# nnanhuang/S3Gaussian

Measured on AMD Instinct MI355X. Metric: train_iters_per_sec, higher is better.
Workload: dtype f32

## Files before the change

include/s3g_loss.h:

```cpp
#ifndef S3G_LOSS_H
#define S3G_LOSS_H
#ifdef __cplusplus
extern "C" {
#endif

#ifndef S3G_SUM_SLOTS
#define S3G_SUM_SLOTS 64
#define S3G_SUM_STRIDE 16
#define S3G_SUM_DOUBLES (S3G_SUM_SLOTS * S3G_SUM_STRIDE)
#endif

int s3g_ssim_forward(int C, int H, int W, const float* img1, const float* img2, double* ssim_sum, float* dm_dmu1,
                     float* dm_dsigma1_sq, float* dm_dsigma12, void* stream);

int s3g_ssim_backward(int C, int H, int W, const float* img1, const float* img2, const float* dm_dmu1,
                      const float* dm_dsigma1_sq, const float* dm_dsigma12, const float* dL_dmean, float* dL_dimg1,
                      void* stream);

typedef struct s3g_plane_reg_desc {
  const float* plane;
  float* grad;
  int H, W;
  float w_smooth, w_l1;
} s3g_plane_reg_desc;

#define S3G_MAX_REG_PLANES 48
int s3g_plane_regulation(int nplanes, const s3g_plane_reg_desc* planes, double* value, void* stream);

int s3g_scale_unless_one(float* x, size_t n, const float* scale , void* stream);

int s3g_pixel_losses_forward(int H, int W, const float* image, const float* gt_image, const float* depth,
                             const float* gt_depth, const float* feat, const float* gt_feat, float max_depth,
                             double* sums, void* stream);

int s3g_pixel_losses_combine(int H, int W, const double* sums, double* totals, float w_l1, float w_depth, float w_ssim,
                             float w_feat, float* loss, void* stream);

int s3g_pixel_losses_backward(int H, int W, const float* image, const float* gt_image, const float* depth,
                              const float* gt_depth, const float* feat, const float* gt_feat, float max_depth,
                              const double* totals, const float* g, float w_l1, float w_depth, float w_feat,
                              float* g_image, int accumulate_image, float* g_depth, float* g_feat, void* stream);

#ifdef __cplusplus
}
#endif
#endif
```

s3gaussian_amd/_lib.py:

```python
from __future__ import annotations

import ctypes as C
import os
import subprocess

_HERE = os.path.dirname(os.path.abspath(__file__))
LIB_PATH = os.environ.get("S3G_LIB_PATH") or os.path.join(_HERE, "lib", "libs3g.so")
CSRC_DIR = os.path.join(_HERE, "csrc")

ABI_VERSION = 16

RESIZE_FN = C.CFUNCTYPE(C.c_void_p, C.c_void_p, C.c_size_t)


class RasterInputs(C.Structure):
    _fields_ = [
        ("P", C.c_int), ("D", C.c_int), ("M", C.c_int), ("width", C.c_int), ("height", C.c_int),
        ("background", C.c_void_p), ("means3D", C.c_void_p), ("shs", C.c_void_p), ("colors_precomp", C.c_void_p),
        ("opacities", C.c_void_p), ("scales", C.c_void_p), ("scale_modifier", C.c_float), ("rotations", C.c_void_p),
        ("cov3D_precomp", C.c_void_p), ("viewmatrix", C.c_void_p), ("projmatrix", C.c_void_p), ("cam_pos", C.c_void_p),
        ("tan_fovx", C.c_float), ("tan_fovy", C.c_float), ("prefiltered", C.c_int), ("debug", C.c_int),
    ]


# ... 89 lines not shown
    return _torch.cuda.current_stream().cuda_stream


class _NullContext:
    __slots__ = ()

    def __enter__(self):
        return None

    def __exit__(self, *exc):
        return False


_NULL = _NullContext()


def on_device(dev):
    global _torch, _raw_stream, _cur_device
    if _torch is None:
        _torch, _raw_stream, _cur_device = _bind_fast_paths()
    if _cur_device is not None and getattr(dev, "index", None) is not None and _cur_device() == dev.index:
        return _NULL
    return _torch.cuda.device(dev)


def check(code: int) -> None:
    if code != 0:
        msg = lib().s3g_last_error().decode("utf-8", "replace")
        if code == 1:
            raise Exception(msg)
        raise RuntimeError(f"libs3g error {code}: {msg}")


EXPORTED_SYMBOLS = ["s3g_raster_forward", "s3g_raster_forward_reuse", "s3g_raster_forward_decompose", "s3g_raster_forward2", "s3g_raster_forward_async", "s3g_raster_arena_bytes", "s3g_adam_step_guarded", "s3g_raster_backward", "s3g_raster_backward_workspace_bytes", "s3g_raster_backward2", "s3g_raster_backward2_workspace_bytes", "s3g_hexplane_forward_workspace_bytes", "s3g_knn_workspace_bytes", "s3g_knn_mean_dist2", "s3g_hexplane_forward", "s3g_hexplane_backward", "s3g_hexplane_backward_algo", "s3g_hexplane_backward_workspace_bytes", "s3g_hexplane_backward_scratch_rows", "s3g_hexplane_debug_walk_mask", "s3g_hexplane_set_deterministic", "s3g_hexplane_get_deterministic", "s3g_hexplane_sort_state_words", "s3g_profile_enable", "s3g_profile_read", "s3g_ssim_forward", "s3g_ssim_backward", "s3g_plane_regulation", "s3g_scale_unless_one", "s3g_pixel_losses_forward", "s3g_pixel_losses_combine", "s3g_pixel_losses_backward", "s3g_glue_forward", "s3g_glue_backward", "s3g_deform_mlp_forward", "s3g_deform_mlp_backward", "s3g_deform_mlp_backward_ordered", "s3g_deform_mlp_wgrad_partial_bytes", "s3g_deform_mlp_stash_bytes", "s3g_deform_mlp_pack_bytes", "s3g_deform_mlp_set_arithmetic", "s3g_deform_mlp_get_arithmetic", "s3g_deform_infer", "s3g_deform_infer_split", "s3g_deform_infer_workspace_bytes", "s3g_adam_step", "s3g_densify_stats", "s3g_densify_stats_guarded", "s3g_density_count_words", "s3g_density_classify_densify", "s3g_density_classify_prune", "s3g_density_scan", "s3g_density_apply", "s3g_density_reset_opacity", "s3g_image_metrics_workspace_bytes", "s3g_image_metrics", "s3g_scene_flow_workspace_bytes", "s3g_scene_flow_colors", "s3g_frame_workspace_bytes", "s3g_frame_tiles", "s3g_split_count_words", "s3g_split_workspace_bytes", "s3g_split_classify", "s3g_split_mask_offsets", "s3g_split_pack_rows", "s3g_raster_backward_accum", "s3g_raster_backward2_accum", "s3g_mark_visible", "s3g_raster_set_exact_cull", "s3g_raster_get_exact_cull", "s3g_raster_set_bin_band", "s3g_raster_set_backward_wave_bounds", "s3g_last_error", "s3g_abi_version"]
```

s3gaussian_amd/csrc/ssim.hip:

```cpp
#include "common.hpp"

#include "../../include/s3g_loss.h"

namespace s3g {

constexpr int SS_T = 16, SS_R = 5, SS_H = SS_T + 2 * SS_R;

struct SsimWindow {
  float g[11];
};
static SsimWindow make_window() {
  SsimWindow w;
  float s = 0.f;
  for (int x = 0; x < 11; x++) {
    w.g[x] = (float)exp(-(double)((x - 5) * (x - 5)) / (2.0 * 1.5 * 1.5));
    s += w.g[x];
  }
  for (int x = 0; x < 11; x++) w.g[x] /= s;
  return w;
}

__global__ void __launch_bounds__(256) ssim_forward_kernel(int C, int H, int W, const float* __restrict__ img1,
                                                           const float* __restrict__ img2, const SsimWindow win,
                                                           double* __restrict__ ssim_sum, float* __restrict__ m_mu1,
                                                           float* __restrict__ m_s11, float* __restrict__ m_s12) {
  __shared__ float t1[SS_H][SS_H + 1], t2[SS_H][SS_H + 1];
  __shared__ float hb[5][SS_H][SS_T + 1];
  __shared__ float red[4];
  const int c = blockIdx.z, x0 = blockIdx.x * SS_T, y0 = blockIdx.y * SS_T;
  const int tid = threadIdx.x, lx = tid & 15, ly = tid >> 4;
  const size_t plane = (size_t)c * H * W;
  for (int i = tid; i < SS_H * SS_H; i += 256) {
    const int r = i / SS_H, q = i - r * SS_H;
    const int gy = y0 + r - SS_R, gx = x0 + q - SS_R;
    const bool in = gy >= 0 && gy < H && gx >= 0 && gx < W;
    t1[r][q] = in ? img1[plane + (size_t)gy * W + gx] : 0.f;
    t2[r][q] = in ? img2[plane + (size_t)gy * W + gx] : 0.f;
  }
  __syncthreads();
  for (int i = tid; i < SS_H * SS_T; i += 256) {
    const int r = i / SS_T, q = i - r * SS_T;
    float a = 0.f, b = 0.f, aa = 0.f, bb = 0.f, ab = 0.f;
#pragma unroll
    for (int k = 0; k < 11; k++) {
      const float w = win.g[k], u = t1[r][q + k], v = t2[r][q + k];
      a += w * u; b += w * v; aa += w * (u * u); bb += w * (v * v); ab += w * (u * v);
    }
    hb[0][r][q] = a; hb[1][r][q] = b; hb[2][r][q] = aa; hb[3][r][q] = bb; hb[4][r][q] = ab;
  }
  __syncthreads();
  float mu1 = 0.f, mu2 = 0.f, e11 = 0.f, e22 = 0.f, e12 = 0.f;
#pragma unroll
  for (int k = 0; k < 11; k++) {
    const float w = win.g[k];
    mu1 += w * hb[0][ly + k][lx]; mu2 += w * hb[1][ly + k][lx]; e11 += w * hb[2][ly + k][lx];
    e22 += w * hb[3][ly + k][lx]; e12 += w * hb[4][ly + k][lx];
  }
  const int gx = x0 + lx, gy = y0 + ly;
  float val = 0.f;
  if (gx < W && gy < H) {
    const float C1 = 0.01f * 0.01f, C2 = 0.03f * 0.03f;
    const float mu1_sq = mu1 * mu1, mu2_sq = mu2 * mu2, mu12 = mu1 * mu2;
    const float s11 = e11 - mu1_sq, s22 = e22 - mu2_sq, s12 = e12 - mu12;
    const float a = 2.f * mu12 + C1, b = 2.f * s12 + C2, cc = mu1_sq + mu2_sq + C1, d = s11 + s22 + C2;
    const float inv = 1.f / (cc * d);
    val = (a * b) * inv;
    const float dm_ds11 = -val / d;
    const float dm_ds12 = 2.f * a * inv;
    const float dm_dmu1 = 2.f * mu2 * b * inv - 2.f * mu1 * val / cc + dm_ds11 * (-2.f * mu1) + dm_ds12 * (-mu2);
    const size_t o = plane + (size_t)gy * W + gx;
    m_mu1[o] = dm_dmu1; m_s11[o] = dm_ds11; m_s12[o] = dm_ds12;
  }
  for (int off = 32; off >= 1; off >>= 1) val += __shfl_xor(val, off);
  if ((tid & 63) == 0) red[tid >> 6] = val;
  __syncthreads();
  if (tid == 0) {
    const unsigned b = blockIdx.x + gridDim.x * (blockIdx.y + gridDim.y * blockIdx.z);
    atomicAdd(&ssim_sum[(b % S3G_SUM_SLOTS) * S3G_SUM_STRIDE], (double)(red[0] + red[1] + red[2] + red[3]));
  }
}

__global__ void __launch_bounds__(256) ssim_backward_kernel(int C, int H, int W, const float* __restrict__ img1,
                                                            const float* __restrict__ img2, const SsimWindow win,
                                                            const float* __restrict__ m_mu1, const float* __restrict__ m_s11,
                                                            const float* __restrict__ m_s12, const float* __restrict__ dL_dmean,
                                                            float* __restrict__ dL_dimg1) {
  __shared__ float t[3][SS_H][SS_H + 1];
  __shared__ float hb[3][SS_H][SS_T + 1];
  const int c = blockIdx.z, x0 = blockIdx.x * SS_T, y0 = blockIdx.y * SS_T;
  const int tid = threadIdx.x, lx = tid & 15, ly = tid >> 4;
  const size_t plane = (size_t)c * H * W;
  for (int i = tid; i < SS_H * SS_H; i += 256) {
    const int r = i / SS_H, q = i - r * SS_H;
    const int gy = y0 + r - SS_R, gx = x0 + q - SS_R;
    const bool in = gy >= 0 && gy < H && gx >= 0 && gx < W;
    const size_t o = plane + (size_t)gy * W + gx;
    t[0][r][q] = in ? m_mu1[o] : 0.f;
    t[1][r][q] = in ? m_s11[o] : 0.f;
    t[2][r][q] = in ? m_s12[o] : 0.f;
  }
  __syncthreads();
  for (int i = tid; i < SS_H * SS_T; i += 256) {
    const int r = i / SS_T, q = i - r * SS_T;
    float a = 0.f, b = 0.f, d = 0.f;
#pragma unroll
    for (int k = 0; k < 11; k++) {
      const float w = win.g[k];
      a += w * t[0][r][q + k]; b += w * t[1][r][q + k]; d += w * t[2][r][q + k];
    }
    hb[0][r][q] = a; hb[1][r][q] = b; hb[2][r][q] = d;
  }
  __syncthreads();
  float A = 0.f, B = 0.f, D = 0.f;
#pragma unroll
  for (int k = 0; k < 11; k++) {
    const float w = win.g[k];
    A += w * hb[0][ly + k][lx]; B += w * hb[1][ly + k][lx]; D += w * hb[2][ly + k][lx];
  }
  const int gx = x0 + lx, gy = y0 + ly;
  if (gx < W && gy < H) {
    const size_t o = plane + (size_t)gy * W + gx;
    const float scale = dL_dmean[0] / (float)((size_t)C * H * W);
    dL_dimg1[o] = scale * (A + 2.f * img1[o] * B + img2[o] * D);
  }
}

}

using namespace s3g;

extern "C" int s3g_ssim_forward(int C, int H, int W, const float* img1, const float* img2, double* ssim_sum, float* dm_dmu1,
                                float* dm_dsigma1_sq, float* dm_dsigma12, void* stream_) {
  if (C <= 0 || H <= 0 || W <= 0 || !img1 || !img2 || !ssim_sum || !dm_dmu1 || !dm_dsigma1_sq || !dm_dsigma12) {
    set_error("s3g_ssim_forward: bad argument");
    return S3G_ERR_INVALID_ARG;
  }
  static const SsimWindow win = make_window();
  dim3 grid((W + SS_T - 1) / SS_T, (H + SS_T - 1) / SS_T, C);
  hipLaunchKernelGGL(ssim_forward_kernel, grid, dim3(256), 0, (hipStream_t)stream_, C, H, W, img1, img2, win, ssim_sum,
                     dm_dmu1, dm_dsigma1_sq, dm_dsigma12);
  S3G_HIP_CHECK(hipGetLastError());
  return S3G_OK;
}

extern "C" int s3g_ssim_backward(int C, int H, int W, const float* img1, const float* img2, const float* dm_dmu1,
                                 const float* dm_dsigma1_sq, const float* dm_dsigma12, const float* dL_dmean,
                                 float* dL_dimg1, void* stream_) {
  if (C <= 0 || H <= 0 || W <= 0 || !img1 || !img2 || !dm_dmu1 || !dm_dsigma1_sq || !dm_dsigma12 || !dL_dmean || !dL_dimg1) {
    set_error("s3g_ssim_backward: bad argument");
    return S3G_ERR_INVALID_ARG;
  }
  static const SsimWindow win = make_window();
  dim3 grid((W + SS_T - 1) / SS_T, (H + SS_T - 1) / SS_T, C);
  hipLaunchKernelGGL(ssim_backward_kernel, grid, dim3(256), 0, (hipStream_t)stream_, C, H, W, img1, img2, win, dm_dmu1,
                     dm_dsigma1_sq, dm_dsigma12, dL_dmean, dL_dimg1);
  S3G_HIP_CHECK(hipGetLastError());
  return S3G_OK;
}

namespace s3g {
struct PixelLossArgs {
  int HW;
  const float *image, *gt_image, *depth, *gt_depth, *feat, *gt_feat;
  float max_depth;
  double* sums;
  const float* g;
  float w_l1, w_depth, w_feat;
  float *g_image, *g_depth, *g_feat;
  int accumulate_image;
};

__device__ __forceinline__ double block_sum(double v, double* part) {
  for (int o = 32; o > 0; o >>= 1) v += __shfl_xor(v, o);
  __syncthreads();
  if ((threadIdx.x & 63) == 0) part[threadIdx.x >> 6] = v;
  __syncthreads();
  return part[0] + part[1] + part[2] + part[3];
}

__global__ void __launch_bounds__(256) pixel_loss_forward_kernel(const PixelLossArgs a) {
  __shared__ double part[4];
  float l1 = 0.f, dsq = 0.f, cnt = 0.f, fsq = 0.f;
  for (int i = blockIdx.x * 256 + threadIdx.x; i < a.HW; i += gridDim.x * 256) {
    if (a.image != nullptr) {
#pragma unroll
      for (int c = 0; c < 3; c++) l1 += fabsf(a.image[(size_t)c * a.HW + i] - a.gt_image[(size_t)c * a.HW + i]);
    }
    if (a.depth != nullptr) {
// ... 229 lines not shown
```

s3gaussian_amd/losses.py:

```python
from __future__ import annotations

import ctypes as C

import torch

from . import _lib

_bound = False
SUM_DOUBLES = 64 * 16


def _bind():
    global _bound
    L = _lib.lib()
    if not _bound:
        vp = C.c_void_p
        L.s3g_ssim_forward.restype = C.c_int
        L.s3g_ssim_forward.argtypes = [C.c_int, C.c_int, C.c_int, vp, vp, vp, vp, vp, vp, vp]
        L.s3g_ssim_backward.restype = C.c_int
        L.s3g_ssim_backward.argtypes = [C.c_int, C.c_int, C.c_int, vp, vp, vp, vp, vp, vp, vp, vp]
        L.s3g_pixel_losses_forward.restype = C.c_int
        L.s3g_pixel_losses_forward.argtypes = [C.c_int, C.c_int, vp, vp, vp, vp, vp, vp, C.c_float, vp, vp]
        L.s3g_pixel_losses_combine.restype = C.c_int
        L.s3g_pixel_losses_combine.argtypes = [C.c_int, C.c_int, vp, vp, C.c_float, C.c_float, C.c_float, C.c_float, vp, vp]
        L.s3g_pixel_losses_backward.restype = C.c_int
        L.s3g_pixel_losses_backward.argtypes = ([C.c_int, C.c_int, vp, vp, vp, vp, vp, vp, C.c_float, vp, vp, C.c_float,
                                                 C.c_float, C.c_float, vp, C.c_int, vp, vp, vp])
        _bound = True
    return L


class _SSIM(torch.autograd.Function):
    @staticmethod
    def forward(ctx, img1, img2):
        if not img1.is_cuda:
            raise RuntimeError(f"ssim: images must live on the GPU (got {img1.device}); no CPU fallback")
        L = _bind()
        a = img1.detach().reshape(-1, img1.shape[-2], img1.shape[-1]).contiguous().float()
        b = img2.detach().reshape(-1, img2.shape[-2], img2.shape[-1]).contiguous().float()
        if a.shape != b.shape:
            raise RuntimeError("ssim: shape mismatch")
        Cn, H, W = a.shape
        total = torch.zeros(SUM_DOUBLES, dtype=torch.float64, device=a.device)
        maps = torch.empty((3, Cn, H, W), dtype=torch.float32, device=a.device)
        with _lib.on_device(a.device):
            _lib.check(L.s3g_ssim_forward(Cn, H, W, a.data_ptr(), b.data_ptr(), total.data_ptr(), maps[0].data_ptr(),
                                          maps[1].data_ptr(), maps[2].data_ptr(), _lib.stream_ptr()))
        ctx.save_for_backward(a, b, maps)
        ctx.shape = img1.shape
        return (total.sum() / float(Cn * H * W)).float()

    @staticmethod
    def backward(ctx, g):
        a, b, maps = ctx.saved_tensors
        L = _bind()
        Cn, H, W = a.shape
        g = g.detach().reshape(1).contiguous().float()
        out = torch.empty_like(a)
        with _lib.on_device(a.device):
            _lib.check(L.s3g_ssim_backward(Cn, H, W, a.data_ptr(), b.data_ptr(), maps[0].data_ptr(), maps[1].data_ptr(),
                                           maps[2].data_ptr(), g.data_ptr(), out.data_ptr(),
                                           _lib.stream_ptr()))
        return out.view(ctx.shape), None


def ssim(img1: torch.Tensor, img2: torch.Tensor, window_size: int = 11, size_average: bool = True) -> torch.Tensor:
    if window_size != 11 or not size_average:
        raise NotImplementedError("only the reference's call signature ssim(img1, img2) is accelerated")
    return _SSIM.apply(img1, img2)


class _PhotometricLoss(torch.autograd.Function):

    @staticmethod
    def forward(ctx, image, gt_image, depth, gt_depth, feat, gt_feat, w_ssim, w_depth, w_feat, max_depth):
        if not image.is_cuda:
            raise RuntimeError(f"photometric_loss: images must live on the GPU (got {image.device}); no CPU fallback")
        L = _bind()
        c = lambda t: None if t is None else t.detach().contiguous().float()
        img, gt = c(image), c(gt_image)
        if img.dim() != 3 or img.shape[0] != 3 or gt.shape != img.shape:
            raise RuntimeError("photometric_loss expects image and gt_image of shape [3,H,W]")
        _, H, W = img.shape
        dev = img.device
        w_ssim, w_depth, w_feat = float(w_ssim), float(w_depth), float(w_feat)
        dep, gdep = (c(depth), c(gt_depth)) if (depth is not None and w_depth != 0.0) else (None, None)
        ft, gft = (c(feat), c(gt_feat)) if (feat is not None and w_feat != 0.0) else (None, None)
        for a, b, n in ((dep, gdep, H * W), (ft, gft, 3 * H * W)):
            if a is not None and (a.numel() != n or b.numel() != n):
                raise RuntimeError("photometric_loss: depth must have H*W and feat 3*H*W elements, like their targets")
        sums = torch.zeros(5 * SUM_DOUBLES + 5, dtype=torch.float64, device=dev)
        totals = sums[5 * SUM_DOUBLES:]
        maps = torch.empty((3, 3, H, W), dtype=torch.float32, device=dev) if w_ssim != 0.0 else None
        loss = torch.empty((), dtype=torch.float32, device=dev)
        p = lambda t: None if t is None else t.data_ptr()
        with _lib.on_device(dev):
            st = _lib.stream_ptr()
            if maps is not None:
                _lib.check(L.s3g_ssim_forward(3, H, W, p(img), p(gt), p(sums), p(maps[0]), p(maps[1]), p(maps[2]), st))
            _lib.check(L.s3g_pixel_losses_forward(H, W, p(img), p(gt), p(dep), p(gdep), p(ft), p(gft), float(max_depth),
                                                  p(sums), st))
            _lib.check(L.s3g_pixel_losses_combine(H, W, p(sums), p(totals), 1.0, w_depth if dep is not None else 0.0, w_ssim,
                                                  w_feat if ft is not None else 0.0, p(loss), st))
        ctx.save_for_backward(img, gt, *(t for t in (dep, gdep, ft, gft, maps) if t is not None), totals)
        ctx.cfg = (H, W, dep is not None, ft is not None, maps is not None, w_ssim, w_depth, w_feat, float(max_depth),
                   None if depth is None else depth.shape, None if feat is None else feat.shape, image.shape)
        return loss

    @staticmethod
    def backward(ctx, g):
        H, W, has_d, has_f, has_s, w_ssim, w_depth, w_feat, max_depth, dshape, fshape, ishape = ctx.cfg
        saved = list(ctx.saved_tensors)
        img, gt = saved[0], saved[1]
        k = 2
        dep = gdep = ft = gft = maps = None
        if has_d:
            dep, gdep = saved[k], saved[k + 1]
            k += 2
        if has_f:
            ft, gft = saved[k], saved[k + 1]
            k += 2
        if has_s:
            maps = saved[k]
            k += 1
        sums = saved[k]
        L = _bind()
        dev = img.device
        g = g.detach().reshape(1).contiguous().float()
        g_img = torch.empty_like(img)
        g_dep = torch.empty_like(dep) if has_d else None
        g_ft = torch.empty_like(ft) if has_f else None
        p = lambda t: None if t is None else t.data_ptr()
        with _lib.on_device(dev):
            st = _lib.stream_ptr()
            if has_s:
                gs = g * (-w_ssim)
                _lib.check(L.s3g_ssim_backward(3, H, W, p(img), p(gt), p(maps[0]), p(maps[1]), p(maps[2]), p(gs), p(g_img), st))
            _lib.check(L.s3g_pixel_losses_backward(H, W, p(img), p(gt), p(dep), p(gdep), p(ft), p(gft), max_depth, p(sums), p(g),
                                                   1.0, w_depth, w_feat, p(g_img), int(has_s), p(g_dep), p(g_ft), st))
        return (g_img.view(ishape), None, g_dep.view(dshape) if has_d else None, None,
                g_ft.view(fshape) if has_f else None, None, None, None, None, None)


def photometric_loss(image, gt_image, depth=None, gt_depth=None, feat=None, gt_feat=None, lambda_dssim=0.0,
                     lambda_depth=0.0, lambda_feat=0.0, max_depth=80.0):
    return _PhotometricLoss.apply(image, gt_image, depth, gt_depth, feat, gt_feat, lambda_dssim, lambda_depth, lambda_feat,
                                  max_depth)


class _PixelTerms(torch.autograd.Function):

    @staticmethod
    def forward(ctx, image, gt_image, depth, gt_depth, feat, gt_feat, w_l1, w_depth, w_feat, max_depth):
        first = next(t for t in (image, depth, feat) if t is not None)
        if not first.is_cuda:
            raise RuntimeError(f"pixel_terms: images must live on the GPU (got {first.device}); no CPU fallback")
        L = _bind()
        c = lambda t: None if t is None else t.detach().contiguous().float()
        img, gt, dep, gdep, ft, gft = c(image), c(gt_image), c(depth), c(gt_depth), c(feat), c(gt_feat)
        H, W = first.shape[-2], first.shape[-1]
        for a, b, n, name in ((img, gt, 3 * H * W, "image"), (dep, gdep, H * W, "depth"), (ft, gft, 3 * H * W, "feat")):
            if (a is None) != (b is None) or (a is not None and (a.numel() != n or b.numel() != n)):
                raise RuntimeError(f"pixel_terms: {name} and its target must both be given, {n} elements each")
        dev = first.device
        sums = torch.zeros(5 * SUM_DOUBLES + 5, dtype=torch.float64, device=dev)
        totals = sums[5 * SUM_DOUBLES:]
        loss = torch.empty((), dtype=torch.float32, device=dev)
        p = lambda t: None if t is None else t.data_ptr()
        wl, wd, wf = (float(w_l1) if img is not None else 0.0, float(w_depth) if dep is not None else 0.0,
                      float(w_feat) if ft is not None else 0.0)
        with _lib.on_device(dev):
            st = _lib.stream_ptr()
            _lib.check(L.s3g_pixel_losses_forward(H, W, p(img), p(gt), p(dep), p(gdep), p(ft), p(gft), float(max_depth), p(sums), st))
            _lib.check(L.s3g_pixel_losses_combine(H, W, p(sums), p(totals), wl, wd, 0.0, wf, p(loss), st))
        ctx.save_for_backward(*(t for t in (img, gt, dep, gdep, ft, gft) if t is not None), totals)
        ctx.cfg = (H, W, img is not None, dep is not None, ft is not None, wl, wd, wf, float(max_depth),
                   None if image is None else image.shape, None if depth is None else depth.shape, None if feat is None else feat.shape)
        return loss

    @staticmethod
    def backward(ctx, g):
        H, W, has_i, has_d, has_f, wl, wd, wf, max_depth, ishape, dshape, fshape = ctx.cfg
        saved = list(ctx.saved_tensors)
        img = gt = dep = gdep = ft = gft = None
        k = 0
        if has_i:
            img, gt = saved[k], saved[k + 1]
            k += 2
        if has_d:
            dep, gdep = saved[k], saved[k + 1]
            k += 2
        if has_f:
            ft, gft = saved[k], saved[k + 1]
            k += 2
        totals = saved[k]
        L = _bind()
        g = g.detach().reshape(1).contiguous().float()
        need = ctx.needs_input_grad
        g_img = torch.empty_like(img) if (has_i and need[0]) else None
        g_dep = torch.empty_like(dep) if (has_d and need[2]) else None
        g_ft = torch.empty_like(ft) if (has_f and need[4]) else None
        p = lambda t: None if t is None else t.data_ptr()
        with _lib.on_device(totals.device):
            _lib.check(L.s3g_pixel_losses_backward(H, W, p(img), p(gt), p(dep), p(gdep), p(ft), p(gft), max_depth, p(totals), p(g),
                                                   wl, wd, wf, p(g_img), 0, p(g_dep), p(g_ft), _lib.stream_ptr()))
        return (None if g_img is None else g_img.view(ishape), None, None if g_dep is None else g_dep.view(dshape), None,
                None if g_ft is None else g_ft.view(fshape), None, None, None, None, None)


def pixel_terms(image=None, gt_image=None, depth=None, gt_depth=None, feat=None, gt_feat=None, w_l1=0.0, w_depth=0.0,
                w_feat=0.0, max_depth=80.0):
    if image is None and depth is None and feat is None:
        raise RuntimeError("pixel_terms: nothing to do")
    return _PixelTerms.apply(image, gt_image, depth, gt_depth, feat, gt_feat, w_l1, w_depth, w_feat, max_depth)


class _PlaneRegDesc(C.Structure):
    _fields_ = [("plane", C.c_void_p), ("grad", C.c_void_p), ("H", C.c_int), ("W", C.c_int), ("w_smooth", C.c_float),
                ("w_l1", C.c_float)]


class _PlaneRegulation(torch.autograd.Function):
    @staticmethod
    def forward(ctx, weights, *planes):
        L = _lib.lib()
        L.s3g_plane_regulation.restype = C.c_int
        L.s3g_plane_regulation.argtypes = [C.c_int, C.POINTER(_PlaneRegDesc), C.c_void_p, C.c_void_p]
        dev = planes[0].device
        if not planes[0].is_cuda:
            raise RuntimeError("plane regulation: planes must live on the GPU; no CPU fallback")
        grads = [torch.empty_like(p) for p in planes]
        descs = (_PlaneRegDesc * len(planes))()
        for i, (p, g, (ws, wl)) in enumerate(zip(planes, grads, weights)):
            if p.dim() != 4 or p.shape[1] != 32 or not p.is_contiguous(memory_format=torch.channels_last):
# ... 48 lines not shown
```

Before: 142.2.

## Rewrite SSIM as wave-per-strip sliding window and fuse with pixel losses

Replaces the 16x16 tiled SSIM kernels with a strip kernel in which each wavefront walks down a 64-column strip. It keeps horizontal blur results in an 11-row register ring, so the halo rows are not reloaded and blurred again for every tile. The photometric loss forward and backward now call new fused entry points that compute the L1, depth and feature terms in the same pass as SSIM, removing separate kernel launches and repeated image reads. The cost is heavy register use from the ring, which may lower occupancy, plus wave-level LDS fences.

Result: faster. 147.6, median of 6 (+3.7%).

```diff
diff --git a/include/s3g_loss.h b/include/s3g_loss.h
--- a/include/s3g_loss.h
+++ b/include/s3g_loss.h
@@ -41,6 +41,16 @@
                               const double* totals, const float* g, float w_l1, float w_depth, float w_feat,
                               float* g_image, int accumulate_image, float* g_depth, float* g_feat, void* stream);
 
+int s3g_photometric_forward(int H, int W, const float* image, const float* gt_image, const float* depth,
+                            const float* gt_depth, const float* feat, const float* gt_feat, float max_depth, double* sums,
+                            float* dm_dmu1, float* dm_dsigma1_sq, float* dm_dsigma12, void* stream);
+
+int s3g_photometric_backward(int H, int W, const float* image, const float* gt_image, const float* depth,
+                             const float* gt_depth, const float* feat, const float* gt_feat, float max_depth,
+                             const float* dm_dmu1, const float* dm_dsigma1_sq, const float* dm_dsigma12,
+                             const double* totals, const float* g, float w_ssim, float w_l1, float w_depth, float w_feat,
+                             float* g_image, float* g_depth, float* g_feat, void* stream);
+
 #ifdef __cplusplus
 }
 #endif
diff --git a/s3gaussian_amd/_lib.py b/s3gaussian_amd/_lib.py
--- a/s3gaussian_amd/_lib.py
+++ b/s3gaussian_amd/_lib.py
@@ -145,4 +145,4 @@
         raise RuntimeError(f"libs3g error {code}: {msg}")
 
 
-EXPORTED_SYMBOLS = ["s3g_raster_forward", "s3g_raster_forward_reuse", "s3g_raster_forward_decompose", "s3g_raster_forward2", "s3g_raster_forward_async", "s3g_raster_arena_bytes", "s3g_adam_step_guarded", "s3g_raster_backward", "s3g_raster_backward_workspace_bytes", "s3g_raster_backward2", "s3g_raster_backward2_workspace_bytes", "s3g_hexplane_forward_workspace_bytes", "s3g_knn_workspace_bytes", "s3g_knn_mean_dist2", "s3g_hexplane_forward", "s3g_hexplane_backward", "s3g_hexplane_backward_algo", "s3g_hexplane_backward_workspace_bytes", "s3g_hexplane_backward_scratch_rows", "s3g_hexplane_debug_walk_mask", "s3g_hexplane_set_deterministic", "s3g_hexplane_get_deterministic", "s3g_hexplane_sort_state_words", "s3g_profile_enable", "s3g_profile_read", "s3g_ssim_forward", "s3g_ssim_backward", "s3g_plane_regulation", "s3g_scale_unless_one", "s3g_pixel_losses_forward", "s3g_pixel_losses_combine", "s3g_pixel_losses_backward", "s3g_glue_forward", "s3g_glue_backward", "s3g_deform_mlp_forward", "s3g_deform_mlp_backward", "s3g_deform_mlp_backward_ordered", "s3g_deform_mlp_wgrad_partial_bytes", "s3g_deform_mlp_stash_bytes", "s3g_deform_mlp_pack_bytes", "s3g_deform_mlp_set_arithmetic", "s3g_deform_mlp_get_arithmetic", "s3g_deform_infer", "s3g_deform_infer_split", "s3g_deform_infer_workspace_bytes", "s3g_adam_step", "s3g_densify_stats", "s3g_densify_stats_guarded", "s3g_density_count_words", "s3g_density_classify_densify", "s3g_density_classify_prune", "s3g_density_scan", "s3g_density_apply", "s3g_density_reset_opacity", "s3g_image_metrics_workspace_bytes", "s3g_image_metrics", "s3g_scene_flow_workspace_bytes", "s3g_scene_flow_colors", "s3g_frame_workspace_bytes", "s3g_frame_tiles", "s3g_split_count_words", "s3g_split_workspace_bytes", "s3g_split_classify", "s3g_split_mask_offsets", "s3g_split_pack_rows", "s3g_raster_backward_accum", "s3g_raster_backward2_accum", "s3g_mark_visible", "s3g_raster_set_exact_cull", "s3g_raster_get_exact_cull", "s3g_raster_set_bin_band", "s3g_raster_set_backward_wave_bounds", "s3g_last_error", "s3g_abi_version"]
+EXPORTED_SYMBOLS = ["s3g_raster_forward", "s3g_raster_forward_reuse", "s3g_raster_forward_decompose", "s3g_raster_forward2", "s3g_raster_forward_async", "s3g_raster_arena_bytes", "s3g_adam_step_guarded", "s3g_raster_backward", "s3g_raster_backward_workspace_bytes", "s3g_raster_backward2", "s3g_raster_backward2_workspace_bytes", "s3g_hexplane_forward_workspace_bytes", "s3g_knn_workspace_bytes", "s3g_knn_mean_dist2", "s3g_hexplane_forward", "s3g_hexplane_backward", "s3g_hexplane_backward_algo", "s3g_hexplane_backward_workspace_bytes", "s3g_hexplane_backward_scratch_rows", "s3g_hexplane_debug_walk_mask", "s3g_hexplane_set_deterministic", "s3g_hexplane_get_deterministic", "s3g_hexplane_sort_state_words", "s3g_profile_enable", "s3g_profile_read", "s3g_ssim_forward", "s3g_ssim_backward", "s3g_plane_regulation", "s3g_scale_unless_one", "s3g_pixel_losses_forward", "s3g_pixel_losses_combine", "s3g_pixel_losses_backward", "s3g_photometric_forward", "s3g_photometric_backward", "s3g_glue_forward", "s3g_glue_backward", "s3g_deform_mlp_forward", "s3g_deform_mlp_backward", "s3g_deform_mlp_backward_ordered", "s3g_deform_mlp_wgrad_partial_bytes", "s3g_deform_mlp_stash_bytes", "s3g_deform_mlp_pack_bytes", "s3g_deform_mlp_set_arithmetic", "s3g_deform_mlp_get_arithmetic", "s3g_deform_infer", "s3g_deform_infer_split", "s3g_deform_infer_workspace_bytes", "s3g_adam_step", "s3g_densify_stats", "s3g_densify_stats_guarded", "s3g_density_count_words", "s3g_density_classify_densify", "s3g_density_classify_prune", "s3g_density_scan", "s3g_density_apply", "s3g_density_reset_opacity", "s3g_image_metrics_workspace_bytes", "s3g_image_metrics", "s3g_scene_flow_workspace_bytes", "s3g_scene_flow_colors", "s3g_frame_workspace_bytes", "s3g_frame_tiles", "s3g_split_count_words", "s3g_split_workspace_bytes", "s3g_split_classify", "s3g_split_mask_offsets", "s3g_split_pack_rows", "s3g_raster_backward_accum", "s3g_raster_backward2_accum", "s3g_mark_visible", "s3g_raster_set_exact_cull", "s3g_raster_get_exact_cull", "s3g_raster_set_bin_band", "s3g_raster_set_backward_wave_bounds", "s3g_last_error", "s3g_abi_version"]
diff --git a/s3gaussian_amd/csrc/ssim.hip b/s3gaussian_amd/csrc/ssim.hip
--- a/s3gaussian_amd/csrc/ssim.hip
+++ b/s3gaussian_amd/csrc/ssim.hip
@@ -4,7 +4,11 @@
 
 namespace s3g {
 
-constexpr int SS_T = 16, SS_R = 5, SS_H = SS_T + 2 * SS_R;
+constexpr int SS_R = 5;
+constexpr int SS_SW = 64;
+constexpr int SS_RH = 21;
+constexpr int SS_WAVES = 8;
+constexpr int SS_PITCH = SS_SW + 2 * SS_R + 6;
 
 struct SsimWindow {
   float g[11];
@@ -20,108 +24,313 @@
   return w;
 }
 
-__global__ void __launch_bounds__(256) ssim_forward_kernel(int C, int H, int W, const float* __restrict__ img1,
-                                                           const float* __restrict__ img2, const SsimWindow win,
-                                                           double* __restrict__ ssim_sum, float* __restrict__ m_mu1,
-                                                           float* __restrict__ m_s11, float* __restrict__ m_s12) {
-  __shared__ float t1[SS_H][SS_H + 1], t2[SS_H][SS_H + 1];
-  __shared__ float hb[5][SS_H][SS_T + 1];
-  __shared__ float red[4];
-  const int c = blockIdx.z, x0 = blockIdx.x * SS_T, y0 = blockIdx.y * SS_T;
-  const int tid = threadIdx.x, lx = tid & 15, ly = tid >> 4;
-  const size_t plane = (size_t)c * H * W;
-  for (int i = tid; i < SS_H * SS_H; i += 256) {
-    const int r = i / SS_H, q = i - r * SS_H;
-    const int gy = y0 + r - SS_R, gx = x0 + q - SS_R;
-    const bool in = gy >= 0 && gy < H && gx >= 0 && gx < W;
-    t1[r][q] = in ? img1[plane + (size_t)gy * W + gx] : 0.f;
-    t2[r][q] = in ? img2[plane + (size_t)gy * W + gx] : 0.f;
-  }
-  __syncthreads();
-  for (int i = tid; i < SS_H * SS_T; i += 256) {
-    const int r = i / SS_T, q = i - r * SS_T;
-    float a = 0.f, b = 0.f, aa = 0.f, bb = 0.f, ab = 0.f;
-#pragma unroll
-    for (int k = 0; k < 11; k++) {
-      const float w = win.g[k], u = t1[r][q + k], v = t2[r][q + k];
-      a += w * u; b += w * v; aa += w * (u * u); bb += w * (v * v); ab += w * (u * v);
-    }
-    hb[0][r][q] = a; hb[1][r][q] = b; hb[2][r][q] = aa; hb[3][r][q] = bb; hb[4][r][q] = ab;
-  }
-  __syncthreads();
-  float mu1 = 0.f, mu2 = 0.f, e11 = 0.f, e22 = 0.f, e12 = 0.f;
-#pragma unroll
-  for (int k = 0; k < 11; k++) {
-    const float w = win.g[k];
-    mu1 += w * hb[0][ly + k][lx]; mu2 += w * hb[1][ly + k][lx]; e11 += w * hb[2][ly + k][lx];
-    e22 += w * hb[3][ly + k][lx]; e12 += w * hb[4][ly + k][lx];
-  }
-  const int gx = x0 + lx, gy = y0 + ly;
-  float val = 0.f;
-  if (gx < W && gy < H) {
-    const float C1 = 0.01f * 0.01f, C2 = 0.03f * 0.03f;
-    const float mu1_sq = mu1 * mu1, mu2_sq = mu2 * mu2, mu12 = mu1 * mu2;
-    const float s11 = e11 - mu1_sq, s22 = e22 - mu2_sq, s12 = e12 - mu12;
-    const float a = 2.f * mu12 + C1, b = 2.f * s12 + C2, cc = mu1_sq + mu2_sq + C1, d = s11 + s22 + C2;
-    const float inv = 1.f / (cc * d);
-    val = (a * b) * inv;
-    const float dm_ds11 = -val / d;
-    const float dm_ds12 = 2.f * a * inv;
-    const float dm_dmu1 = 2.f * mu2 * b * inv - 2.f * mu1 * val / cc + dm_ds11 * (-2.f * mu1) + dm_ds12 * (-mu2);
-    const size_t o = plane + (size_t)gy * W + gx;
-    m_mu1[o] = dm_dmu1; m_s11[o] = dm_ds11; m_s12[o] = dm_ds12;
-  }
-  for (int off = 32; off >= 1; off >>= 1) val += __shfl_xor(val, off);
-  if ((tid & 63) == 0) red[tid >> 6] = val;
-  __syncthreads();
-  if (tid == 0) {
-    const unsigned b = blockIdx.x + gridDim.x * (blockIdx.y + gridDim.y * blockIdx.z);
-    atomicAdd(&ssim_sum[(b % S3G_SUM_SLOTS) * S3G_SUM_STRIDE], (double)(red[0] + red[1] + red[2] + red[3]));
-  }
-}
-
-__global__ void __launch_bounds__(256) ssim_backward_kernel(int C, int H, int W, const float* __restrict__ img1,
-                                                            const float* __restrict__ img2, const SsimWindow win,
-                                                            const float* __restrict__ m_mu1, const float* __restrict__ m_s11,
-                                                            const float* __restrict__ m_s12, const float* __restrict__ dL_dmean,
-                                                            float* __restrict__ dL_dimg1) {
-  __shared__ float t[3][SS_H][SS_H + 1];
-  __shared__ float hb[3][SS_H][SS_T + 1];
-  const int c = blockIdx.z, x0 = blockIdx.x * SS_T, y0 = blockIdx.y * SS_T;
-  const int tid = threadIdx.x, lx = tid & 15, ly = tid >> 4;
-  const size_t plane = (size_t)c * H * W;
-  for (int i = tid; i < SS_H * SS_H; i += 256) {
-    const int r = i / SS_H, q = i - r * SS_H;
-    const int gy = y0 + r - SS_R, gx = x0 + q - SS_R;
-    const bool in = gy >= 0 && gy < H && gx >= 0 && gx < W;
-    const size_t o = plane + (size_t)gy * W + gx;
-    t[0][r][q] = in ? m_mu1[o] : 0.f;
-    t[1][r][q] = in ? m_s11[o] : 0.f;
-    t[2][r][q] = in ? m_s12[o] : 0.f;
-  }
-  __syncthreads();
-  for (int i = tid; i < SS_H * SS_T; i += 256) {
-    const int r = i / SS_T, q = i - r * SS_T;
-    float a = 0.f, b = 0.f, d = 0.f;
-#pragma unroll
-    for (int k = 0; k < 11; k++) {
-      const float w = win.g[k];
-      a += w * t[0][r][q + k]; b += w * t[1][r][q + k]; d += w * t[2][r][q + k];
-    }
-    hb[0][r][q] = a; hb[1][r][q] = b; hb[2][r][q] = d;
-  }
-  __syncthreads();
-  float A = 0.f, B = 0.f, D = 0.f;
-#pragma unroll
-  for (int k = 0; k < 11; k++) {
-    const float w = win.g[k];
-    A += w * hb[0][ly + k][lx]; B += w * hb[1][ly + k][lx]; D += w * hb[2][ly + k][lx];
-  }
-  const int gx = x0 + lx, gy = y0 + ly;
-  if (gx < W && gy < H) {
-    const size_t o = plane + (size_t)gy * W + gx;
-    const float scale = dL_dmean[0] / (float)((size_t)C * H * W);
-    dL_dimg1[o] = scale * (A + 2.f * img1[o] * B + img2[o] * D);
+struct Strip {
+  int c, x0, y0;
+  int nrows;
+};
+__device__ __forceinline__ Strip locate_strip(int C, int H, int W) {
+  const int sx = (W + SS_SW - 1) / SS_SW, sy = (H + SS_RH - 1) / SS_RH;
+  const int wave = __builtin_amdgcn_readfirstlane((int)(blockIdx.x * SS_WAVES + (threadIdx.x >> 6)));
+  Strip s;
+  s.c = wave / (sx * sy);
+  const int rem = wave - s.c * (sx * sy), ys = rem / sx;
+  s.x0 = (rem - ys * sx) * SS_SW;
+  s.y0 = ys * SS_RH;
+  s.nrows = s.c < C ? min(SS_RH, H - s.y0) + 2 * SS_R : 0;
+  return s;
+}
+static int strip_workgroups(int C, int H, int W) {
+  const int waves = C * ((W + SS_SW - 1) / SS_SW) * ((H + SS_RH - 1) / SS_RH);
+  return (waves + SS_WAVES - 1) / SS_WAVES;
+}
+
+struct LaneCols {
+  int gx, hx, hj;
+  bool colok, hok, halo;
+};
+__device__ __forceinline__ LaneCols lane_columns(int lane, int x0, int W) {
+  LaneCols q;
+  q.gx = x0 + lane;
+  q.colok = q.gx < W;
+  q.halo = lane < 2 * SS_R;
+  q.hx = lane < SS_R ? x0 - SS_R + lane : x0 + SS_SW - SS_R + lane;
+  q.hj = lane < SS_R ? lane : SS_SW + lane;
+  q.hok = q.halo && q.hx >= 0 && q.hx < W;
+  return q;
+}
+
+__device__ __forceinline__ void wave_lds_fence() {
+  __builtin_amdgcn_fence(__ATOMIC_ACQ_REL, "wavefront");
+  __builtin_amdgcn_wave_barrier();
+}
+
+struct SsimFwdArgs {
+  int C, H, W;
+  const float *img1, *img2;
+  SsimWindow win;
+  double* sums;
+  float *m_mu1, *m_s11, *m_s12;
+  const float *depth, *gt_depth, *feat, *gt_feat;
+  float max_depth;
+};
+
+template <int P>
+struct RingSlot {
+  static constexpr int value = P;
+};
+
+__device__ __forceinline__ double wave_sum(double v) {
+  for (int o = 32; o > 0; o >>= 1) v += __shfl_xor(v, o);
+  return v;
+}
+
+template <bool FUSED>
+__global__ void __launch_bounds__(SS_WAVES * 64) ssim_strip_forward_kernel(const SsimFwdArgs a) {
+  __shared__ float stage[SS_WAVES][2][SS_PITCH];
+  const Strip s = locate_strip(a.C, a.H, a.W);
+  if (s.nrows == 0) return;
+  const int H = a.H, W = a.W, lane = threadIdx.x & 63;
+  const LaneCols q = lane_columns(lane, s.x0, W);
+  float* const bu = stage[threadIdx.x >> 6][0];
+  float* const bv = stage[threadIdx.x >> 6][1];
+  const size_t plane = (size_t)s.c * H * W;
+  const float *p1 = a.img1 + plane, *p2 = a.img2 + plane;
+  const bool do_depth = FUSED && s.c == 0 && a.depth != nullptr, do_feat = FUSED && a.feat != nullptr;
+
+  struct Row {
+    float u, v, hu, hv, d, gd, f, gf;
+  };
+  auto fetch = [&](int r, Row& n) {
+    const int gy = s.y0 - SS_R + r;
+    if (r < s.nrows && gy >= 0 && gy < H) {
+      const size_t ro = (size_t)gy * W;
+      n.u = q.colok ? p1[ro + q.gx] : 0.f;
+      n.v = q.colok ? p2[ro + q.gx] : 0.f;
+      n.hu = q.hok ? p1[ro + q.hx] : 0.f;
+      n.hv = q.hok ? p2[ro + q.hx] : 0.f;
+      if (FUSED && r >= SS_R && r < s.nrows - SS_R && q.colok) {
+        if (do_depth) { n.d = a.depth[ro + q.gx]; n.gd = a.gt_depth[ro + q.gx]; }
+        if (do_feat) { n.f = a.feat[plane + ro + q.gx]; n.gf = a.gt_feat[plane + ro + q.gx]; }
+      }
+    }
+  };
+
+  float ring[11][5];
+  double vsum = 0.0, l1 = 0.0, dsq = 0.0, fsq = 0.0;
+  float cnt = 0.f;
+  const Row kNoRow = {0.f, 0.f, 0.f, 0.f, 0.f, 0.f, 0.f, 0.f};
+  Row cur = kNoRow;
+  fetch(0, cur);
+  auto step = [&](auto slot, int r) {
+    constexpr int p = decltype(slot)::value;
+    {
+      if (r >= s.nrows) return;
+      const int gy = s.y0 - SS_R + r;
+      const bool rowin = gy >= 0 && gy < H;
+      if (rowin) {
+        bu[lane + SS_R] = cur.u;
+        bv[lane + SS_R] = cur.v;
+        if (q.halo) { bu[q.hj] = cur.hu; bv[q.hj] = cur.hv; }
+      }
+      Row nxt = kNoRow;
+      fetch(r + 1, nxt);
+      wave_lds_fence();
+      float ha = 0.f, hb = 0.f, haa = 0.f, hbb = 0.f, hab = 0.f;
+      if (rowin) {
+#pragma unroll
+        for (int k = 0; k < 11; k++) {
+          const float w = a.win.g[k], u = bu[lane + k], v = bv[lane + k];
+          ha += w * u; hb += w * v; haa += w * (u * u); hbb += w * (v * v); hab += w * (u * v);
+        }
+      }
+      wave_lds_fence();
+      ring[p][0] = ha; ring[p][1] = hb; ring[p][2] = haa; ring[p][3] = hbb; ring[p][4] = hab;
+      if (FUSED && r >= SS_R && r < s.nrows - SS_R && q.colok) {
+        l1 += (double)fabsf(cur.u - cur.v);
+        if (do_depth) {
+          const float gd = cur.gd;
+          if (gd > 0.01f && gd < a.max_depth) {
+            const float cp = fminf(fmaxf(cur.d / a.max_depth, 0.f), 1.f), cg = fminf(fmaxf(gd / a.max_depth, 0.f), 1.f);
+            dsq += (double)((cp - cg) * (cp - cg));
+            cnt += 1.f;
+          }
+        }
+        if (do_feat) {
+          const float d = cur.f - cur.gf;
+          fsq += (double)(d * d);
+        }
+      }
+      if (r >= 2 * SS_R) {
+        float mu1 = 0.f, mu2 = 0.f, e11 = 0.f, e22 = 0.f, e12 = 0.f;
+#pragma unroll
+        for (int k = 0; k < 11; k++) {
+          const float w = a.win.g[k];
+          const float* h = ring[(p + 1 + k) % 11];
+          mu1 += w * h[0]; mu2 += w * h[1]; e11 += w * h[2]; e22 += w * h[3]; e12 += w * h[4];
+        }
+        if (q.colok) {
+          const float C1 = 0.01f * 0.01f, C2 = 0.03f * 0.03f;
+          const float mu1_sq = mu1 * mu1, mu2_sq = mu2 * mu2, mu12 = mu1 * mu2;
+          const float s11 = e11 - mu1_sq, s22 = e22 - mu2_sq, s12 = e12 - mu12;
+          const float aa = 2.f * mu12 + C1, b = 2.f * s12 + C2, cc = mu1_sq + mu2_sq + C1, d = s11 + s22 + C2;
+          const float inv = 1.f / (cc * d);
+          const float val = (aa * b) * inv;
+          const float dm_ds11 = -val / d;
+          const float dm_ds12 = 2.f * aa * inv;
+          const float dm_dmu1 = 2.f * mu2 * b * inv - 2.f * mu1 * val / cc + dm_ds11 * (-2.f * mu1) + dm_ds12 * (-mu2);
+          const size_t o = plane + (size_t)(gy - SS_R) * W + q.gx;
+          a.m_mu1[o] = dm_dmu1; a.m_s11[o] = dm_ds11; a.m_s12[o] = dm_ds12;
+          vsum += (double)val;
+        }
+      }
+      cur = nxt;
+    }
+  };
+  for (int base = 0; base < s.nrows; base += 11) {
+    step(RingSlot<0>{}, base); step(RingSlot<1>{}, base + 1); step(RingSlot<2>{}, base + 2); step(RingSlot<3>{}, base + 3);
+    step(RingSlot<4>{}, base + 4); step(RingSlot<5>{}, base + 5); step(RingSlot<6>{}, base + 6); step(RingSlot<7>{}, base + 7);
+    step(RingSlot<8>{}, base + 8); step(RingSlot<9>{}, base + 9); step(RingSlot<10>{}, base + 10);
+  }
+  vsum = wave_sum(vsum);
+  const unsigned wave = blockIdx.x * SS_WAVES + (threadIdx.x >> 6);
+  double* slot = a.sums + (wave % S3G_SUM_SLOTS) * S3G_SUM_STRIDE;
+  if (FUSED) {
+    const double s1 = wave_sum(l1), s2 = wave_sum(dsq), s3 = wave_sum((double)cnt), s4 = wave_sum(fsq);
+    if (lane == 0) {
+      atomicAdd(&slot[1 * S3G_SUM_DOUBLES], s1);
+      if (do_depth) { atomicAdd(&slot[2 * S3G_SUM_DOUBLES], s2); atomicAdd(&slot[3 * S3G_SUM_DOUBLES], s3); }
+      if (do_feat) atomicAdd(&slot[4 * S3G_SUM_DOUBLES], s4);
+    }
+  }
+  if (lane == 0) atomicAdd(&slot[0], vsum);
+}
+
+struct SsimBwdArgs {
+  int C, H, W;
+  const float *img1, *img2;
+  SsimWindow win;
+  const float *m_mu1, *m_s11, *m_s12;
+  const float* g;
+  float gmul;
+  float* g_image;
+  const float *depth, *gt_depth, *feat, *gt_feat;
+  float max_depth;
+  const double* totals;
+  float w_l1, w_depth, w_feat;
+  float *g_depth, *g_feat;
+};
+
+template <bool FUSED>
+__global__ void __launch_bounds__(SS_WAVES * 64) ssim_strip_backward_kernel(const SsimBwdArgs a) {
+  __shared__ float stage[SS_WAVES][3][SS_PITCH];
+  const Strip s = locate_strip(a.C, a.H, a.W);
+  if (s.nrows == 0) return;
+  const int H = a.H, W = a.W, lane = threadIdx.x & 63;
+  const LaneCols q = lane_columns(lane, s.x0, W);
+  float* const b0 = stage[threadIdx.x >> 6][0];
+  float* const b1 = stage[threadIdx.x >> 6][1];
+  float* const b2 = stage[threadIdx.x >> 6][2];
+  const size_t plane = (size_t)s.c * H * W;
+  const float *m0 = a.m_mu1 + plane, *m1 = a.m_s11 + plane, *m2 = a.m_s12 + plane;
+  const float *p1 = a.img1 + plane, *p2 = a.img2 + plane;
+  const bool do_depth = FUSED && s.c == 0 && a.g_depth != nullptr, do_feat = FUSED && a.g_feat != nullptr;
+  const float scale = (a.g[0] * a.gmul) / (float)((size_t)a.C * H * W);
+  float k_l1 = 0.f, k_feat = 0.f, k_depth = 0.f;
+  if (FUSED) {
+    const float g = a.g[0];
+    const int HW = H * W;
+    k_l1 = g * a.w_l1 / (3.0f * (float)HW);
+    k_feat = g * a.w_feat * 2.0f / (3.0f * (float)HW);
+    k_depth = a.g_depth != nullptr ? g * a.w_depth * 2.0f / ((float)a.totals[3] * a.max_depth) : 0.f;
+  }
+
+  struct Row {
+    float t0, t1, t2, h0, h1, h2;
+    float x1, x2, d, gd, f, gf;
+  };
+  auto fetch = [&](int r, Row& n) {
+    const int gy = s.y0 - SS_R + r;
+    if (r < s.nrows && gy >= 0 && gy < H) {
+      const size_t ro = (size_t)gy * W;
+      n.t0 = q.colok ? m0[ro + q.gx] : 0.f;
+      n.t1 = q.colok ? m1[ro + q.gx] : 0.f;
+      n.t2 = q.colok ? m2[ro + q.gx] : 0.f;
+      n.h0 = q.hok ? m0[ro + q.hx] : 0.f;
+      n.h1 = q.hok ? m1[ro + q.hx] : 0.f;
+      n.h2 = q.hok ? m2[ro + q.hx] : 0.f;
+    }
+    if (r >= 2 * SS_R && r < s.nrows && q.colok) {
+      const size_t oo = (size_t)(gy - SS_R) * W + q.gx;
+      n.x1 = p1[oo];
+      n.x2 = p2[oo];
+      if (do_depth) { n.d = a.depth[oo]; n.gd = a.gt_depth[oo]; }
+      if (do_feat) { n.f = a.feat[plane + oo]; n.gf = a.gt_feat[plane + oo]; }
+    }
+  };
+
+  float ring[11][3];
+  const Row kNoRow = {0.f, 0.f, 0.f, 0.f, 0.f, 0.f, 0.f, 0.f, 0.f, 0.f, 0.f, 0.f};
+  Row cur = kNoRow;
+  fetch(0, cur);
+  auto step = [&](auto slot, int r) {
+    constexpr int p = decltype(slot)::value;
+    {
+      if (r >= s.nrows) return;
+      const int gy = s.y0 - SS_R + r;
+      const bool rowin = gy >= 0 && gy < H;
+      if (rowin) {
+        b0[lane + SS_R] = cur.t0;
+        b1[lane + SS_R] = cur.t1;
+        b2[lane + SS_R] = cur.t2;
+        if (q.halo) { b0[q.hj] = cur.h0; b1[q.hj] = cur.h1; b2[q.hj] = cur.h2; }
+      }
+      Row nxt = kNoRow;
+      fetch(r + 1, nxt);
+      wave_lds_fence();
+      float ha = 0.f, hb = 0.f, hd = 0.f;
+      if (rowin) {
+#pragma unroll
+        for (int k = 0; k < 11; k++) {
+          const float w = a.win.g[k];
+          ha += w * b0[lane + k]; hb += w * b1[lane + k]; hd += w * b2[lane + k];
+        }
+      }
+      wave_lds_fence();
+      ring[p][0] = ha; ring[p][1] = hb; ring[p][2] = hd;
+      if (r >= 2 * SS_R) {
+        float A = 0.f, B = 0.f, D = 0.f;
+#pragma unroll
+        for (int k = 0; k < 11; k++) {
+          const float w = a.win.g[k];
+          const float* h = ring[(p + 1 + k) % 11];
+          A += w * h[0]; B += w * h[1]; D += w * h[2];
+        }
+        if (q.colok) {
+          const size_t oo = (size_t)(gy - SS_R) * W + q.gx;
+          float out = scale * (A + 2.f * cur.x1 * B + cur.x2 * D);
+          if (FUSED) {
+            const float d = cur.x1 - cur.x2;
+            const float v = d > 0.f ? k_l1 : (d < 0.f ? -k_l1 : 0.f);
+            out = out + v;
+            if (do_depth) {
+              const float gd = cur.gd, x = cur.d / a.max_depth;
+              float gv = 0.f;
+              if (gd > 0.01f && gd < a.max_depth && x >= 0.f && x <= 1.f)
+                gv = k_depth * (x - fminf(fmaxf(gd / a.max_depth, 0.f), 1.f));
+              a.g_depth[oo] = gv;
+            }
+            if (do_feat) a.g_feat[plane + oo] = k_feat * (cur.f - cur.gf);
+          }
+          a.g_image[plane + oo] = out;
+        }
+      }
+      cur = nxt;
+    }
+  };
+  for (int base = 0; base < s.nrows; base += 11) {
+    step(RingSlot<0>{}, base); step(RingSlot<1>{}, base + 1); step(RingSlot<2>{}, base + 2); step(RingSlot<3>{}, base + 3);
+    step(RingSlot<4>{}, base + 4); step(RingSlot<5>{}, base + 5); step(RingSlot<6>{}, base + 6); step(RingSlot<7>{}, base + 7);
+    step(RingSlot<8>{}, base + 8); step(RingSlot<9>{}, base + 9); step(RingSlot<10>{}, base + 10);
   }
 }
 
@@ -136,9 +345,12 @@
     return S3G_ERR_INVALID_ARG;
   }
   static const SsimWindow win = make_window();
-  dim3 grid((W + SS_T - 1) / SS_T, (H + SS_T - 1) / SS_T, C);
-  hipLaunchKernelGGL(ssim_forward_kernel, grid, dim3(256), 0, (hipStream_t)stream_, C, H, W, img1, img2, win, ssim_sum,
-                     dm_dmu1, dm_dsigma1_sq, dm_dsigma12);
+  SsimFwdArgs a;
+  memset(&a, 0, sizeof a);
+  a.C = C; a.H = H; a.W = W; a.img1 = img1; a.img2 = img2; a.win = win; a.sums = ssim_sum;
+  a.m_mu1 = dm_dmu1; a.m_s11 = dm_dsigma1_sq; a.m_s12 = dm_dsigma12;
+  hipLaunchKernelGGL(ssim_strip_forward_kernel<false>, dim3(strip_workgroups(C, H, W)), dim3(SS_WAVES * 64), 0,
+                     (hipStream_t)stream_, a);
   S3G_HIP_CHECK(hipGetLastError());
   return S3G_OK;
 }
@@ -151,9 +363,55 @@
     return S3G_ERR_INVALID_ARG;
   }
   static const SsimWindow win = make_window();
-  dim3 grid((W + SS_T - 1) / SS_T, (H + SS_T - 1) / SS_T, C);
-  hipLaunchKernelGGL(ssim_backward_kernel, grid, dim3(256), 0, (hipStream_t)stream_, C, H, W, img1, img2, win, dm_dmu1,
-                     dm_dsigma1_sq, dm_dsigma12, dL_dmean, dL_dimg1);
+  SsimBwdArgs a;
+  memset(&a, 0, sizeof a);
+  a.C = C; a.H = H; a.W = W; a.img1 = img1; a.img2 = img2; a.win = win;
+  a.m_mu1 = dm_dmu1; a.m_s11 = dm_dsigma1_sq; a.m_s12 = dm_dsigma12; a.g = dL_dmean; a.gmul = 1.0f; a.g_image = dL_dimg1;
+  hipLaunchKernelGGL(ssim_strip_backward_kernel<false>, dim3(strip_workgroups(C, H, W)), dim3(SS_WAVES * 64), 0,
+                     (hipStream_t)stream_, a);
+  S3G_HIP_CHECK(hipGetLastError());
+  return S3G_OK;
+}
+
+extern "C" int s3g_photometric_forward(int H, int W, const float* image, const float* gt_image, const float* depth,
+                                       const float* gt_depth, const float* feat, const float* gt_feat, float max_depth,
+                                       double* sums, float* dm_dmu1, float* dm_dsigma1_sq, float* dm_dsigma12, void* stream_) {
+  if (H <= 0 || W <= 0 || !image || !gt_image || !sums || !dm_dmu1 || !dm_dsigma1_sq || !dm_dsigma12 || (depth && !gt_depth) ||
+      (feat && !gt_feat)) {
+    set_error("s3g_photometric_forward: bad argument");
+    return S3G_ERR_INVALID_ARG;
+  }
+  static const SsimWindow win = make_window();
+  SsimFwdArgs a;
+  memset(&a, 0, sizeof a);
+  a.C = 3; a.H = H; a.W = W; a.img1 = image; a.img2 = gt_image; a.win = win; a.sums = sums;
+  a.m_mu1 = dm_dmu1; a.m_s11 = dm_dsigma1_sq; a.m_s12 = dm_dsigma12;
+  a.depth = depth; a.gt_depth = gt_depth; a.feat = feat; a.gt_feat = gt_feat; a.max_depth = max_depth;
+  hipLaunchKernelGGL(ssim_strip_forward_kernel<true>, dim3(strip_workgroups(3, H, W)), dim3(SS_WAVES * 64), 0,
+                     (hipStream_t)stream_, a);
+  S3G_HIP_CHECK(hipGetLastError());
+  return S3G_OK;
+}
+
+extern "C" int s3g_photometric_backward(int H, int W, const float* image, const float* gt_image, const float* depth,
+                                        const float* gt_depth, const float* feat, const float* gt_feat, float max_depth,
+                                        const float* dm_dmu1, const float* dm_dsigma1_sq, const float* dm_dsigma12,
+                                        const double* totals, const float* g, float w_ssim, float w_l1, float w_depth,
+                                        float w_feat, float* g_image, float* g_depth, float* g_feat, void* stream_) {
+  if (H <= 0 || W <= 0 || !image || !gt_image || !dm_dmu1 || !dm_dsigma1_sq || !dm_dsigma12 || !totals || !g || !g_image ||
+      (g_depth && (!depth || !gt_depth)) || (g_feat && (!feat || !gt_feat))) {
+    set_error("s3g_photometric_backward: bad argument");
+    return S3G_ERR_INVALID_ARG;
+  }
+  static const SsimWindow win = make_window();
+  SsimBwdArgs a;
+  memset(&a, 0, sizeof a);
+  a.C = 3; a.H = H; a.W = W; a.img1 = image; a.img2 = gt_image; a.win = win;
+  a.m_mu1 = dm_dmu1; a.m_s11 = dm_dsigma1_sq; a.m_s12 = dm_dsigma12; a.g = g; a.gmul = -w_ssim; a.g_image = g_image;
+  a.depth = depth; a.gt_depth = gt_depth; a.feat = feat; a.gt_feat = gt_feat; a.max_depth = max_depth; a.totals = totals;
+  a.w_l1 = w_l1; a.w_depth = w_depth; a.w_feat = w_feat; a.g_depth = g_depth; a.g_feat = g_feat;
+  hipLaunchKernelGGL(ssim_strip_backward_kernel<true>, dim3(strip_workgroups(3, H, W)), dim3(SS_WAVES * 64), 0,
+                     (hipStream_t)stream_, a);
   S3G_HIP_CHECK(hipGetLastError());
   return S3G_OK;
 }
diff --git a/s3gaussian_amd/losses.py b/s3gaussian_amd/losses.py
--- a/s3gaussian_amd/losses.py
+++ b/s3gaussian_amd/losses.py
@@ -8,6 +8,8 @@
 
 _bound = False
 SUM_DOUBLES = 64 * 16
+_new_grad = torch.empty_like
+_new_maps = torch.empty
 
 
 def _bind():
@@ -26,6 +28,11 @@
         L.s3g_pixel_losses_backward.restype = C.c_int
         L.s3g_pixel_losses_backward.argtypes = ([C.c_int, C.c_int, vp, vp, vp, vp, vp, vp, C.c_float, vp, vp, C.c_float,
                                                  C.c_float, C.c_float, vp, C.c_int, vp, vp, vp])
+        L.s3g_photometric_forward.restype = C.c_int
+        L.s3g_photometric_forward.argtypes = [C.c_int, C.c_int, vp, vp, vp, vp, vp, vp, C.c_float, vp, vp, vp, vp, vp]
+        L.s3g_photometric_backward.restype = C.c_int
+        L.s3g_photometric_backward.argtypes = ([C.c_int, C.c_int, vp, vp, vp, vp, vp, vp, C.c_float, vp, vp, vp, vp, vp,
+                                                C.c_float, C.c_float, C.c_float, C.c_float, vp, vp, vp, vp])
         _bound = True
     return L
 
@@ -42,7 +49,7 @@
             raise RuntimeError("ssim: shape mismatch")
         Cn, H, W = a.shape
         total = torch.zeros(SUM_DOUBLES, dtype=torch.float64, device=a.device)
-        maps = torch.empty((3, Cn, H, W), dtype=torch.float32, device=a.device)
+        maps = _new_maps((3, Cn, H, W), dtype=torch.float32, device=a.device)
         with _lib.on_device(a.device):
             _lib.check(L.s3g_ssim_forward(Cn, H, W, a.data_ptr(), b.data_ptr(), total.data_ptr(), maps[0].data_ptr(),
                                           maps[1].data_ptr(), maps[2].data_ptr(), _lib.stream_ptr()))
@@ -56,7 +63,7 @@
         L = _bind()
         Cn, H, W = a.shape
         g = g.detach().reshape(1).contiguous().float()
-        out = torch.empty_like(a)
+        out = _new_grad(a)
         with _lib.on_device(a.device):
             _lib.check(L.s3g_ssim_backward(Cn, H, W, a.data_ptr(), b.data_ptr(), maps[0].data_ptr(), maps[1].data_ptr(),
                                            maps[2].data_ptr(), g.data_ptr(), out.data_ptr(),
@@ -91,15 +98,17 @@
                 raise RuntimeError("photometric_loss: depth must have H*W and feat 3*H*W elements, like their targets")
         sums = torch.zeros(5 * SUM_DOUBLES + 5, dtype=torch.float64, device=dev)
         totals = sums[5 * SUM_DOUBLES:]
-        maps = torch.empty((3, 3, H, W), dtype=torch.float32, device=dev) if w_ssim != 0.0 else None
+        maps = _new_maps((3, 3, H, W), dtype=torch.float32, device=dev) if w_ssim != 0.0 else None
         loss = torch.empty((), dtype=torch.float32, device=dev)
         p = lambda t: None if t is None else t.data_ptr()
         with _lib.on_device(dev):
             st = _lib.stream_ptr()
             if maps is not None:
-                _lib.check(L.s3g_ssim_forward(3, H, W, p(img), p(gt), p(sums), p(maps[0]), p(maps[1]), p(maps[2]), st))
-            _lib.check(L.s3g_pixel_losses_forward(H, W, p(img), p(gt), p(dep), p(gdep), p(ft), p(gft), float(max_depth),
-                                                  p(sums), st))
+                _lib.check(L.s3g_photometric_forward(H, W, p(img), p(gt), p(dep), p(gdep), p(ft), p(gft), float(max_depth),
+                                                     p(sums), p(maps[0]), p(maps[1]), p(maps[2]), st))
+            else:
+                _lib.check(L.s3g_pixel_losses_forward(H, W, p(img), p(gt), p(dep), p(gdep), p(ft), p(gft), float(max_depth),
+                                                      p(sums), st))
             _lib.check(L.s3g_pixel_losses_combine(H, W, p(sums), p(totals), 1.0, w_depth if dep is not None else 0.0, w_ssim,
                                                   w_feat if ft is not None else 0.0, p(loss), st))
         ctx.save_for_backward(img, gt, *(t for t in (dep, gdep, ft, gft, maps) if t is not None), totals)
@@ -127,17 +136,19 @@
         L = _bind()
         dev = img.device
         g = g.detach().reshape(1).contiguous().float()
-        g_img = torch.empty_like(img)
-        g_dep = torch.empty_like(dep) if has_d else None
-        g_ft = torch.empty_like(ft) if has_f else None
+        g_img = _new_grad(img)
+        g_dep = _new_grad(dep) if has_d else None
+        g_ft = _new_grad(ft) if has_f else None
         p = lambda t: None if t is None else t.data_ptr()
         with _lib.on_device(dev):
             st = _lib.stream_ptr()
             if has_s:
-                gs = g * (-w_ssim)
-                _lib.check(L.s3g_ssim_backward(3, H, W, p(img), p(gt), p(maps[0]), p(maps[1]), p(maps[2]), p(gs), p(g_img), st))
-            _lib.check(L.s3g_pixel_losses_backward(H, W, p(img), p(gt), p(dep), p(gdep), p(ft), p(gft), max_depth, p(sums), p(g),
-                                                   1.0, w_depth, w_feat, p(g_img), int(has_s), p(g_dep), p(g_ft), st))
+                _lib.check(L.s3g_photometric_backward(H, W, p(img), p(gt), p(dep), p(gdep), p(ft), p(gft), max_depth, p(maps[0]),
+                                                      p(maps[1]), p(maps[2]), p(sums), p(g), w_ssim, 1.0, w_depth, w_feat,
+                                                      p(g_img), p(g_dep), p(g_ft), st))
+            else:
+                _lib.check(L.s3g_pixel_losses_backward(H, W, p(img), p(gt), p(dep), p(gdep), p(ft), p(gft), max_depth, p(sums),
+                                                       p(g), 1.0, w_depth, w_feat, p(g_img), 0, p(g_dep), p(g_ft), st))
         return (g_img.view(ishape), None, g_dep.view(dshape) if has_d else None, None,
                 g_ft.view(fshape) if has_f else None, None, None, None, None, None)
 
@@ -197,9 +208,9 @@
         L = _bind()
         g = g.detach().reshape(1).contiguous().float()
         need = ctx.needs_input_grad
-        g_img = torch.empty_like(img) if (has_i and need[0]) else None
-        g_dep = torch.empty_like(dep) if (has_d and need[2]) else None
-        g_ft = torch.empty_like(ft) if (has_f and need[4]) else None
+        g_img = _new_grad(img) if (has_i and need[0]) else None
+        g_dep = _new_grad(dep) if (has_d and need[2]) else None
+        g_ft = _new_grad(ft) if (has_f and need[4]) else None
         p = lambda t: None if t is None else t.data_ptr()
         with _lib.on_device(totals.device):
             _lib.check(L.s3g_pixel_losses_backward(H, W, p(img), p(gt), p(dep), p(gdep), p(ft), p(gft), max_depth, p(totals), p(g),
```
